# pengfeidip/pytorch-faster-rcnn

Measured on AMD Instinct MI355X. Metric: img/s FasterRCNN_R50_FPN 1000x600 fwd+loss, higher is better.
Workload: dtype f32; 1 GPU; configs/faster_rcnn_r50_fpn.py (BASELINE config 2) forward_train; conv_algorithms=MIOpen benchmarked (warmup, at most 32 tuning iterations per solver), trunk=hipGraph replay (backbone + neck + RPN head convs), global_batch=2, imgs_per_gpu=2, image=600x1000 padded 608x1024, parallelism=dp1, sampler=device, mode=fwd

## Files before the change

include/frcnn_amd.h:

```cpp
#ifndef FRCNN_AMD_H
#define FRCNN_AMD_H

#include <stddef.h>
#include <stdint.h>

#ifdef __cplusplus
extern "C" {
#endif

#define FRH_ABI_VERSION 3

#define FRH_OK 0
#define FRH_EINVAL (-1)
#define FRH_EUNSUPPORTED (-2)
#define FRH_ELAUNCH (-3)

#define FRH_MAX_LEVELS 8

int32_t frh_abi_version(void);
const char* frh_last_error(void);

#define FRH_DEVERR_SELECT_BARRIER 1
#define FRH_DEVERR_NMS_COLUMN 2
#define FRH_DEVERR_SAMPLER_BARRIER 4
// ... 213 lines not shown
                         int32_t channels, const float* rois, int64_t num_rois, int32_t pooled_h,
                         int32_t pooled_w, const float* grad_out, const int32_t* argmax, void* stream);

size_t frh_atss_workspace(int32_t batch, int32_t max_gts, int32_t num_levels, int32_t topk,
                          int64_t num_cells);
int32_t frh_atss_assign(int32_t batch, int32_t num_levels, const int32_t* grid_hw,
                        const float* strides, const float* anchors, int64_t anchor_ld,
                        const float* gts, int64_t gt_seg_stride, const int32_t* num_gts,
                        const int64_t* gt_labels, int32_t max_gts, const int32_t* img_hw,
                        int32_t topk, int64_t* cls, float* reg, float* ctr, void* workspace,
                        size_t ws_bytes, void* stream);

int32_t frh_bn_act(const float* x, const float* skip, float* y, const float* gamma,
                   const float* beta, const float* mean, const float* var, float eps,
                   int64_t n, int32_t c, int64_t hw, int32_t relu, void* stream);

int32_t frh_bn_act_maxpool(const float* x, float* y, const float* gamma, const float* beta, const float* mean,
                           const float* var, float eps, int64_t n, int32_t c, int32_t h, int32_t w, void* stream);

int32_t frh_conv1x1_bn_act(const float* x, const float* w, const float* skip, float* y, const float* gamma,
                           const float* beta, const float* mean, const float* var, float eps, int64_t n,
                           int32_t cin, int32_t cout, int64_t hw, int32_t relu, void* stream);

size_t frh_conv3x3_workspace(int32_t cin, int32_t cout);
int32_t frh_conv3x3_bias_act(const float* x, const float* w, const float* bias, float* y, float* workspace,
                             int64_t n, int32_t cin, int32_t cout, int32_t h, int32_t wd, int64_t sn, int64_t sy,
                             int64_t sx, int32_t relu, void* stream);
int32_t frh_conv3x3_bias_act_levels(int32_t num_levels, const void* const* xs, const void* const* weights,
                                    const void* const* biases, void* const* ys, float* workspace,
                                    size_t workspace_bytes, int64_t n, int32_t cin, int32_t cout,
                                    const int32_t* level_hw, const int64_t* level_strides, int32_t relu,
                                    void* stream);

size_t frh_roi_conv3x3_workspace(int32_t cin, int32_t cout);
int32_t frh_roi_conv3x3_bn_act(const float* x, const float* w, float* y, const float* gamma, const float* beta,
                               const float* mean, const float* var, float eps, int64_t r, int32_t cin,
                               int32_t cout, int32_t relu, float* workspace, void* stream);

int32_t frh_fpn_merge_nhwc(const float* lat, const int64_t* lat_strides, const float* bias, const float* up,
                           int32_t up_h, int32_t up_w, float* out, int32_t batch, int32_t channels, int32_t height,
                           int32_t width, void* stream);

size_t frh_bfp_argmax_elems(int32_t num_levels, int32_t refine_level, int32_t batch, int32_t channels,
                            const int32_t* level_hw);
int32_t frh_bfp_fwd(int32_t num_levels, int32_t refine_level, int32_t batch, int32_t channels,
                    const void* const* feats, const int32_t* level_hw, const int64_t* level_strides,
// ... 72 lines not shown
```

pytorch-faster-rcnn_amd/csrc/conv1x1.hip:

```cpp
#include "conv1x1_kernels.h"

using namespace frh;

extern "C" int32_t frh_conv1x1_bn_act(const float* x, const float* w, const float* skip, float* y, const float* gamma,
                                      const float* beta, const float* mean, const float* var, float eps, int64_t n,
                                      int32_t cin, int32_t cout, int64_t hw, int32_t relu, void* stream) {
  return conv1x1_launch(conv1x1_pick_step(cin), x, w, skip, y, gamma, beta, mean, var, eps, n, cin, cout, hw, relu,
                        stream);
}
```

pytorch-faster-rcnn_amd/csrc/conv1x1_kernels.h:

```cpp
#pragma once
#include <math.h>

#include "common.h"

namespace frh {

typedef float f32x16 __attribute__((ext_vector_type(16)));

constexpr int kCxThreads = 256;
constexpr int kCxTile = 64;
constexpr int kCxXcds = 8;

struct Conv1x1Args {
  const float* x;
  const float* w;
  const float* skip;
  float* y;
  const float* gamma;
  const float* beta;
  const float* mean;
  const float* var;
  float eps;
  int cin, cout;
  int64_t hw;
  int mt, pt;
  int64_t total;
  int64_t chunk;
  int relu;
};

template <int BK>
__global__ void __launch_bounds__(kCxThreads) conv1x1_bn_act_kernel(const Conv1x1Args a) {
  constexpr int T = kCxTile, PA = BK + 4, PB = T + 4, HK = BK / 2;
  constexpr int NV = T * (BK / 4) / kCxThreads;
  static_assert(NV == 1 || NV == 2, "staging registers are written out for one or two float4");
  constexpr int A_ROWS = kCxThreads / (BK / 4), B_ROWS = kCxThreads / (T / 4);
  __shared__ __attribute__((aligned(16))) float As[2][T * PA];
  __shared__ __attribute__((aligned(16))) float Bs[2][BK * PB];
  __shared__ float bn_s[T], bn_b[T];

  const int64_t wg = (int64_t)(blockIdx.x % kCxXcds) * a.chunk + blockIdx.x / kCxXcds;
  if (wg >= a.total) return;
  const int m_tile = (int)(wg % a.mt);
  const int64_t rest = wg / a.mt;
  const int p_tile = (int)(rest % a.pt);
  const int64_t img = rest / a.pt;
  const int m0 = m_tile * T;
  const int64_t p0 = (int64_t)p_tile * T;

  const int tid = threadIdx.x;
  const int lane = tid & 63, wave = tid >> 6;
  const int wm = wave >> 1, wn = wave & 1;
  const int h = lane >> 5, j = lane & 31;

  const bool bn = a.mean != nullptr;
  if (bn && tid < T) {
    const int c = m0 + tid;
    const float s = (a.gamma ? a.gamma[c] : 1.0f) / sqrtf(a.var[c] + a.eps);
    bn_s[tid] = s;
    bn_b[tid] = (a.beta ? a.beta[c] : 0.0f) - a.mean[c] * s;
  }

  const int a_row = tid / (BK / 4), a_q = tid % (BK / 4);
  const int b_row = tid / (T / 4), b_q = tid % (T / 4);
  const float* wp = a.w + (int64_t)(m0 + a_row) * a.cin + a_q * 4;
  const bool p_ok = p0 + b_q * 4 < a.hw;
  const float* xp = a.x + (img * a.cin + b_row) * a.hw + p0 + b_q * 4;
  const float4 z4 = make_float4(0.0f, 0.0f, 0.0f, 0.0f);
  float4 ra0, ra1 = z4, rb0 = z4, rb1 = z4;
#define FRH_CX_LOAD(k0)                                                                         \
  do {                                                                                          \
    ra0 = *reinterpret_cast<const float4*>(wp + (k0));                                          \
    if (NV > 1) ra1 = *reinterpret_cast<const float4*>(wp + (int64_t)A_ROWS * a.cin + (k0));    \
    if (p_ok) {                                                                                 \
      rb0 = *reinterpret_cast<const float4*>(xp + (int64_t)(k0)*a.hw);                          \
      if (NV > 1) rb1 = *reinterpret_cast<const float4*>(xp + (int64_t)((k0) + B_ROWS) * a.hw); \
    }                                                                                           \
  } while (0)

  f32x16 acc;
#pragma unroll
  for (int r = 0; r < 16; ++r) acc[r] = 0.0f;

  const int steps = a.cin / BK;
  FRH_CX_LOAD(0);
  for (int t = 0; t < steps; ++t) {
    const int buf = t & 1;
    *reinterpret_cast<float4*>(&As[buf][a_row * PA + a_q * 4]) = ra0;
    if (NV > 1) *reinterpret_cast<float4*>(&As[buf][(a_row + A_ROWS) * PA + a_q * 4]) = ra1;
    *reinterpret_cast<float4*>(&Bs[buf][b_row * PB + b_q * 4]) = rb0;
    if (NV > 1) *reinterpret_cast<float4*>(&Bs[buf][(b_row + B_ROWS) * PB + b_q * 4]) = rb1;
    __syncthreads();
    if (t + 1 < steps) FRH_CX_LOAD((t + 1) * BK);
#pragma unroll
    for (int q = 0; q < HK / 8; ++q) {
      const float* ap = &As[buf][(wm * 32 + j) * PA + h * HK + q * 8];
      const float4 lo = *reinterpret_cast<const float4*>(ap);
      const float4 hi = *reinterpret_cast<const float4*>(ap + 4);
      const float af[8] = {lo.x, lo.y, lo.z, lo.w, hi.x, hi.y, hi.z, hi.w};
      float bf[8];
#pragma unroll
      for (int s = 0; s < 8; ++s) bf[s] = Bs[buf][(h * HK + q * 8 + s) * PB + wn * 32 + j];
#pragma unroll
      for (int s = 0; s < 8; ++s) acc = __builtin_amdgcn_mfma_f32_32x32x2f32(af[s], bf[s], acc, 0, 0, 0);
    }
  }
#undef FRH_CX_LOAD

  const int64_t p = p0 + wn * 32 + j;
  if (p >= a.hw) return;
  const int lrow = wm * 32 + 4 * h;
  const int64_t off = (img * a.cout + m0 + lrow) * a.hw + p;
  float k[16];
  if (a.skip) {
#pragma unroll
    for (int r = 0; r < 16; ++r) k[r] = a.skip[off + (int64_t)((r & 3) + 8 * (r >> 2)) * a.hw];
  }
#pragma unroll
  for (int r = 0; r < 16; ++r) {
    const int lr = lrow + (r & 3) + 8 * (r >> 2);
    float v = acc[r];
    if (bn) v = v * bn_s[lr] + bn_b[lr];
    if (a.skip) v = v + k[r];
    if (a.relu) v = fmaxf(v, 0.0f);
    a.y[off + (int64_t)((r & 3) + 8 * (r >> 2)) * a.hw] = v;
  }
}

inline int conv1x1_pick_step(int32_t cin) { return cin >= 128 && cin % 32 == 0 ? 32 : 16; }

inline int32_t conv1x1_launch(int step, const float* x, const float* w, const float* skip, float* y,
                              const float* gamma, const float* beta, const float* mean, const float* var, float eps,
                              int64_t n, int32_t cin, int32_t cout, int64_t hw, int32_t relu, void* stream) {
  FRH_REQUIRE(n >= 0 && cin >= 1 && cout >= 1 && hw >= 0, "bad sizes");
  if (n == 0 || hw == 0) return FRH_OK;
  FRH_REQUIRE(x && w && y, "null pointer argument");
  FRH_REQUIRE((mean == nullptr) == (var == nullptr), "mean and var must both be given or both be NULL");
  FRH_REQUIRE(hw % 4 == 0, "plane size %lld must be a multiple of 4", (long long)hw);
  FRH_REQUIRE(cin % 16 == 0 && cout % kCxTile == 0, "cin %d must be a multiple of 16 and cout %d of 64", cin, cout);
  FRH_REQUIRE(((uintptr_t)x | (uintptr_t)y | (uintptr_t)skip | (uintptr_t)w) % 16 == 0,
              "tensors must be 16-byte aligned");
  FRH_REQUIRE(y != x && y != skip, "y must not alias x or skip");
  FRH_REQUIRE((step == 16 || step == 32) && cin % step == 0, "step %d does not fit cin %d", step, cin);
  Conv1x1Args a;
  a.x = x, a.w = w, a.skip = skip, a.y = y, a.gamma = gamma, a.beta = beta, a.mean = mean, a.var = var, a.eps = eps;
  a.cin = cin, a.cout = cout, a.hw = hw, a.relu = relu;
  a.mt = cout / kCxTile;
  const int64_t pt = (hw + kCxTile - 1) / kCxTile;
  FRH_REQUIRE(pt < ((int64_t)1 << 31), "too many pixel tiles");
  a.pt = (int)pt;
  a.total = (int64_t)a.mt * pt * n;
  a.chunk = (a.total + kCxXcds - 1) / kCxXcds;
  FRH_REQUIRE(a.chunk * kCxXcds < ((int64_t)1 << 31), "too many blocks");
  const dim3 grid((unsigned)(a.chunk * kCxXcds)), block(kCxThreads);
  if (step == 32)
    hipLaunchKernelGGL((conv1x1_bn_act_kernel<32>), grid, block, 0, as_stream(stream), a);
  else
    hipLaunchKernelGGL((conv1x1_bn_act_kernel<16>), grid, block, 0, as_stream(stream), a);
  return check_launch("frh_conv1x1_bn_act");
}

}
```

pytorch-faster-rcnn_amd/frcnn_amd/_lib.py:

```python
import ctypes
import os

import torch

_HERE = os.path.dirname(os.path.abspath(__file__))
LIB_PATH = os.path.join(_HERE, 'libfrcnn_amd.so')

c_i32, c_i64, c_f32, c_f64 = ctypes.c_int32, ctypes.c_int64, ctypes.c_float, ctypes.c_double
c_u64, c_size, c_vp = ctypes.c_uint64, ctypes.c_size_t, ctypes.c_void_p
P = ctypes.POINTER

SIGNATURES = {
    'frh_abi_version': (c_i32, []),
    'frh_last_error': (ctypes.c_char_p, []),
    'frh_anchor_grid': (c_i32, [c_i32, P(c_i32), P(c_f32), c_vp, c_vp, c_i32, c_i32, c_vp, c_i64, c_vp]),
    'frh_inside_mask': (c_i32, [c_vp, c_i64, c_i32, P(c_i32), P(c_i32), c_i32, c_i32, c_i32, c_i32, c_vp, c_vp]),
    'frh_iou_table': (c_i32, [c_vp, c_i64, c_i64, c_vp, c_i64, c_i64, c_vp, c_vp]),
    'frh_elem_iou': (c_i32, [c_vp, c_i64, c_vp, c_i64, c_i64, c_vp, c_vp]),
    'frh_maxiou_assign_zero_bytes': (c_size, [c_i32, c_i32]),
    'frh_maxiou_assign_workspace': (c_size, [c_i32, c_i32, c_i64]),
    'frh_maxiou_assign': (c_i32, [c_i32, c_vp, c_i64, c_i64, c_vp, c_vp, c_i64, c_vp, c_i64, c_i64, c_vp,
                                  c_f32, c_f32, c_f32, c_vp, c_i64, c_vp, c_i64, c_i64, c_i32, c_vp, c_size,
                                  c_vp]),
    'frh_sample_workspace': (c_size, [c_i32, c_i64]),
# ... 49 lines not shown
    'frh_roi_rows': (c_i32, [c_i32, c_vp, c_i64, c_i64, c_i32, P(c_i64), c_f32, c_i32, c_vp, c_vp, c_vp]),
    'frh_roi_rows_dev': (c_i32, [c_i32, c_vp, c_i64, c_i64, c_vp, c_f32, c_i32, c_vp, c_vp, c_vp]),
    'frh_roi_align_fwd': (c_i32, [c_i32, P(c_vp), P(c_i32), P(c_f32), c_i32, c_i32, c_i32, c_vp, c_vp, c_i64,
                                  c_i32, c_i32, c_i32, c_i32, c_vp, c_vp]),
    'frh_roi_align_bwd': (c_i32, [c_i32, P(c_vp), P(c_i32), P(c_f32), c_i32, c_i32, c_i32, c_vp, c_vp, c_i64,
                                  c_i32, c_i32, c_i32, c_i32, c_vp, c_vp]),
    'frh_roi_align_fwd_strided': (c_i32, [c_i32, P(c_vp), P(c_i32), P(c_i64), P(c_f32), c_i32, c_i32, c_vp,
                                          c_vp, c_i64, c_i32, c_i32, c_i32, c_i32, c_vp, c_vp]),
    'frh_roi_align_fwd_strided_timed': (c_i32, [c_i32, P(c_vp), P(c_i32), P(c_i64), P(c_f32), c_i32, c_i32, c_vp,
                                                c_vp, c_i64, c_i32, c_i32, c_i32, c_i32, c_vp, c_vp, c_vp, c_vp,
                                                c_vp]),
    'frh_roi_align_bwd_strided': (c_i32, [c_i32, P(c_vp), P(c_i32), P(c_i64), P(c_f32), c_i32, c_i32, c_vp,
                                          c_vp, c_i64, c_i32, c_i32, c_i32, c_i32, c_vp, c_vp]),
    'frh_roi_align_bwd_fixed': (c_i32, [c_i32, P(c_vp), P(c_vp), P(c_i32), P(c_i64), P(c_f32), c_i32, c_i32, c_vp,
                                        c_vp, c_i64, c_i32, c_i32, c_i32, c_i32, c_vp, c_vp, c_vp]),
    'frh_roi_pool_fwd': (c_i32, [c_vp, P(c_i64), c_i32, c_i32, c_i32, c_f32, c_vp, c_i64, c_i32, c_i32, c_vp,
                                 c_vp, c_vp]),
    'frh_roi_pool_bwd': (c_i32, [c_vp, P(c_i64), c_i32, c_i32, c_i32, c_vp, c_i64, c_i32, c_i32, c_vp, c_vp,
                                 c_vp]),
    'frh_atss_workspace': (c_size, [c_i32, c_i32, c_i32, c_i32, c_i64]),
    'frh_bn_act': (c_i32, [c_vp, c_vp, c_vp, c_vp, c_vp, c_vp, c_vp, c_f32, c_i64, c_i32, c_i64, c_i32, c_vp]),
    'frh_conv1x1_bn_act': (c_i32, [c_vp, c_vp, c_vp, c_vp, c_vp, c_vp, c_vp, c_vp, c_f32, c_i64, c_i32, c_i32, c_i64, c_i32,
                                   c_vp]),
    'frh_conv3x3_workspace': (c_size, [c_i32, c_i32]),
    'frh_conv3x3_bias_act': (c_i32, [c_vp, c_vp, c_vp, c_vp, c_vp, c_i64, c_i32, c_i32, c_i32, c_i32, c_i64, c_i64, c_i64,
                                     c_i32, c_vp]),
    'frh_conv3x3_bias_act_levels': (c_i32, [c_i32, P(c_vp), P(c_vp), P(c_vp), P(c_vp), c_vp, c_size, c_i64, c_i32, c_i32,
                                            P(c_i32), P(c_i64), c_i32, c_vp]),
    'frh_roi_conv3x3_workspace': (c_size, [c_i32, c_i32]),
    'frh_roi_conv3x3_bn_act': (c_i32, [c_vp, c_vp, c_vp, c_vp, c_vp, c_vp, c_vp, c_f32, c_i64, c_i32, c_i32, c_i32, c_vp,
                                       c_vp]),
    'frh_bn_act_maxpool': (c_i32, [c_vp, c_vp, c_vp, c_vp, c_vp, c_vp, c_f32, c_i64, c_i32, c_i32, c_i32, c_vp]),
    'frh_loss_workspace': (c_size, []),
    'frh_fpn_merge_nhwc': (c_i32, [c_vp, P(c_i64), c_vp, c_vp, c_i32, c_i32, c_vp, c_i32, c_i32, c_i32, c_i32, c_vp]),
    'frh_bfp_argmax_elems': (c_size, [c_i32, c_i32, c_i32, c_i32, P(c_i32)]),
    'frh_bfp_fwd': (c_i32, [c_i32, c_i32, c_i32, c_i32, P(c_vp), P(c_i32), P(c_i64), c_vp, P(c_vp), c_vp, c_i64,
                            c_vp]),
    'frh_bfp_bwd': (c_i32, [c_i32, c_i32, c_i32, c_i32, P(c_vp), P(c_i32), P(c_i64), c_vp, c_i64, c_vp, P(c_vp),
                            c_vp]),
    'frh_bias_act_nhwc': (c_i32, [c_vp, c_vp, c_i64, c_i32, c_i32, c_vp]),
    'frh_image_preprocess': (c_i32, [c_vp, c_i32, P(c_i64), P(c_i32), P(c_i32), P(c_i32), P(c_f32), P(c_f32), c_i32,
                                     c_vp, c_i32, c_i32, c_vp]),
    'frh_cls_loss_fwd': (c_i32, [c_i32, c_vp, c_i64, c_i64, c_i64, c_i64, c_vp, c_i32, c_f32, c_f32, c_vp, c_vp,
                                 c_vp, c_size, c_vp]),
    'frh_cls_loss_bwd': (c_i32, [c_i32, c_vp, c_i64, c_i64, c_i64, c_i64, c_vp, c_i32, c_f32, c_f32, c_vp, c_vp,
                                 c_i64, c_i64, c_vp]),
# ... 87 lines not shown
```

pytorch-faster-rcnn_amd/frcnn_amd/backbones.py:

```python
import logging

import torch
from torch import nn

from .ops import bn_act, bn_act_maxpool, conv1x1_bn_act

_STAGE_BLOCKS = {50: (3, 4, 6, 3), 101: (3, 4, 23, 3), 152: (3, 8, 36, 3)}
_STAGE_WIDTH = (64, 256, 512, 1024, 2048)


def _conv_bn(cin, cout, k, stride=1, pad=0):
    return nn.Conv2d(cin, cout, k, stride=stride, padding=pad, bias=False), nn.BatchNorm2d(cout)


class Bottleneck(nn.Module):

    def __init__(self, in_channels, out_channels, downsample=False):
        super().__init__()
        mid = out_channels // 4
        first_stage = in_channels * 4 == out_channels
        stride = 2 if (downsample and not first_stage) else 1
        self.conv1, self.bn1 = _conv_bn(in_channels, mid, 1)
        self.conv2, self.bn2 = _conv_bn(mid, mid, 3, stride=stride, pad=1)
        self.conv3, self.bn3 = _conv_bn(mid, out_channels, 1)
        self.relu = nn.ReLU(inplace=True)
        self.do_downsample = downsample
        if downsample:
            self.downsample = nn.Sequential(*_conv_bn(in_channels, out_channels, 1, stride=stride))

    def forward(self, x):
        y = conv1x1_bn_act(self.conv1, self.bn1, x)
        y = bn_act(self.conv2(y), self.bn2)
        skip = conv1x1_bn_act(self.downsample[0], self.downsample[1], x, relu=False) if self.do_downsample else x
        return conv1x1_bn_act(self.conv3, self.bn3, y, skip=skip)


class ResNet(nn.Module):
    def __init__(self, depth=50, frozen_stages=1, out_layers=(1, 2, 3, 4), pretrained=True):
        super().__init__()
        if depth not in _STAGE_BLOCKS:
            raise AssertionError('unsupported ResNet depth {}'.format(depth))
        self.depth = depth
        self.pretrained = pretrained
        self.frozen_stages = frozen_stages
        self.out_layers = tuple(out_layers)
        self.conv_cfg = _STAGE_BLOCKS[depth]
        self.conv1, self.bn1 = _conv_bn(3, 64, 7, stride=2, pad=3)
        self.relu = nn.ReLU(inplace=True)
        self.maxpool = nn.MaxPool2d(kernel_size=3, stride=2, padding=1)
        for s, nblk in enumerate(self.conv_cfg):
            cin, cout = _STAGE_WIDTH[s], _STAGE_WIDTH[s + 1]
            blocks = [Bottleneck(cin, cout, True)] + [Bottleneck(cout, cout) for _ in range(nblk - 1)]
            setattr(self, 'layer{}'.format(s + 1), nn.Sequential(*blocks))

    def forward(self, x):
        x = bn_act_maxpool(self.conv1(x), self.bn1, self.maxpool)
        outs = []
# ... 60 lines not shown
```

pytorch-faster-rcnn_amd/frcnn_amd/heads/rpn_head.py:

```python
import logging

import torch
from torch import nn

from .. import ops
from ..bbox import PropBatch
from ..utils import init_module_normal
from .anchor_head import AnchorHead


class LazyPropList(PropBatch):

    def __init__(self, buffer, counts_dev, what='boxes'):
        super().__init__()
        self.buffer = buffer
        self.counts_dev = counts_dev
        self._what = what
        self._n = buffer.shape[0]
        self._done = False

    def _materialise(self):
        if not self._done:
            self._done = True
            counts = self.counts_dev.cpu().tolist()
# ... 20 lines not shown
    def __init__(self, in_channels, feat_channels, anchor_scales=(8,), anchor_ratios=(0.5, 1.0, 2.0),
                 anchor_strides=(4, 8, 16, 32, 64), anchor_center_lt=False, target_means=(0.0, 0.0, 0.0, 0.0),
                 target_stds=(1.0, 1.0, 1.0, 1.0), loss_cls=None, loss_bbox=None):
        self.in_channels = in_channels
        self.feat_channels = feat_channels
        super().__init__(num_classes=2, anchor_scales=anchor_scales, anchor_ratios=anchor_ratios,
                         anchor_strides=anchor_strides, anchor_center_lt=anchor_center_lt,
                         target_means=target_means, target_stds=target_stds, loss_cls=loss_cls,
                         loss_bbox=loss_bbox)
        self.init_layers()

    def init_layers(self):
        self.conv = nn.Conv2d(self.in_channels, self.feat_channels, kernel_size=3, stride=1, padding=1)
        self.relu = nn.ReLU(inplace=True)
        self.classifier = nn.Conv2d(self.feat_channels, self.num_anchors * self.cls_channels, kernel_size=1)
        self.regressor = nn.Conv2d(self.feat_channels, self.num_anchors * 4, kernel_size=1)

    def init_weights(self):
        for m in (self.conv, self.classifier, self.regressor):
            init_module_normal(m, mean=0.0, std=0.01)

    def forward(self, xs):
        hidden = ops.conv3x3_bias_act_levels(self.conv, xs, relu=True)
        return [self.classifier(h) for h in hidden], [self.regressor(h) for h in hidden]

    def predict_bboxes_from_output(self, cls_outs, reg_outs, img_metas, test_cfg):
        with torch.no_grad():
            dev = cls_outs[0].device
            grid_sizes = [tuple(c.shape[-2:]) for c in cls_outs]
            anchors = self._flat_anchors(grid_sizes, dev)
            img_hw = [tuple(float(v) for v in m['img_shape'][:2]) for m in img_metas]
            min_sizes = [float(m['scale_factor'] * test_cfg.min_bbox_size) for m in img_metas]
            boxes, scores, counts = ops.rpn_proposals(
                [c.detach() for c in cls_outs], [r.detach() for r in reg_outs], anchors, self.num_anchors,
                self.cls_channels, self.target_means, self.target_stds, img_hw, min_sizes, int(test_cfg.pre_nms),
                int(test_cfg.post_nms), int(test_cfg.max_num), float(test_cfg.nms_iou))
        props = LazyPropList(boxes, counts, 'boxes')
        scs = LazyPropList(scores, counts, 'scores')
        return [props, scs, [None] * len(img_metas)]

    def predict_single_image(self, level_cls_outs, level_reg_outs, level_anchors, img_meta, test_cfg):
        p, s, _ = self.predict_bboxes_from_output([c.unsqueeze(0) for c in level_cls_outs],
                                                  [r.unsqueeze(0) for r in level_reg_outs], [img_meta], test_cfg)
        return p[0], s[0], None
```

pytorch-faster-rcnn_amd/frcnn_amd/ops.py:

```python
import ctypes
import os
import warnings

import numpy as np
import torch
from torch import nn

from . import _lib
from ._lib import call as _call, ptr, stream_of, i32_array, i64_array, f32_array, ptr_array, workspace


def call(name, *args):
    try:
        _call(name, *args)
    except RuntimeError:
        _drop_zero_workspaces()
        raise


def _drop_zero_workspaces():
    for ws in (_ASSIGN_WS, _SAMPLE_WS, _LOSS_WS):
        ws.clear()


# ... 1027 lines not shown
    return torch.is_grad_enabled() and any(t is not None and t.requires_grad for t in tensors)


_CONV1X1_EXCLUDED = frozenset([(512, 128), (512, 256), (1024, 256), (1024, 512), (2048, 512)])


def conv1x1_fused_ok(conv, bn, x, skip=None):
    if not (x.is_cuda and x.dtype == torch.float32 and x.dim() == 4 and x.is_contiguous()
            and not bn.training and conv.bias is None and conv.weight.dtype == torch.float32
            and conv.kernel_size == (1, 1) and conv.stride == (1, 1) and conv.padding == (0, 0)
            and conv.dilation == (1, 1) and conv.groups == 1 and conv.weight.is_contiguous()):
        return False
    cout, cin, hw = conv.out_channels, conv.in_channels, x.shape[2] * x.shape[3]
    if x.shape[1] != cin or hw % 4 or cin % 16 or cout % 64 or (x.data_ptr() | conv.weight.data_ptr()) % 16 \
            or (cin, cout) in _CONV1X1_EXCLUDED:
        return False
    if skip is not None and not (skip.is_cuda and skip.dtype == torch.float32 and skip.is_contiguous()
                                 and skip.shape == (x.shape[0], cout, x.shape[2], x.shape[3])
                                 and skip.data_ptr() % 16 == 0):
        return False
    return not _needs_grad(x, skip, conv.weight, bn.weight, bn.bias)


def conv1x1_bn_act(conv, bn, x, skip=None, relu=True):
    if not conv1x1_fused_ok(conv, bn, x, skip):
        return bn_act(conv(x), bn, skip=skip, relu=relu)
    n, _, h, w = x.shape
    y = torch.empty(n, conv.out_channels, h, w, dtype=torch.float32, device=x.device)
    call('frh_conv1x1_bn_act', ptr(x), ptr(conv.weight), ptr(skip), ptr(y), ptr(bn.weight), ptr(bn.bias),
         ptr(bn.running_mean), ptr(bn.running_var), float(bn.eps), n, conv.in_channels, conv.out_channels, h * w,
         int(bool(relu)), stream_of(x))
    return y


def roi_conv3x3_fused_ok(conv, bn, x):
    if not (x.is_cuda and x.dtype == torch.float32 and x.dim() == 4 and x.shape[2:] == (7, 7) and x.is_contiguous()
            and not bn.training and bn.running_mean is not None and conv.bias is None and conv.weight.dtype == torch.float32
            and conv.kernel_size == (3, 3) and conv.stride == (1, 1) and conv.padding == (1, 1)
            and conv.dilation == (1, 1) and conv.groups == 1 and conv.padding_mode == 'zeros'
            and conv.weight.is_contiguous()):
        return False
    cout, cin = conv.out_channels, conv.in_channels
    if x.shape[1] != cin or cin % 16 or cout % 64 or (x.data_ptr() | conv.weight.data_ptr()) % 16:
        return False
    return not _needs_grad(x, conv.weight, bn.weight, bn.bias)


def roi_conv3x3_bn_act(conv, bn, x, relu=True):
    if not roi_conv3x3_fused_ok(conv, bn, x):
        y = bn(conv(x))
        return torch.relu(y) if relu else y
    r = x.shape[0]
    y = torch.empty(r, conv.out_channels, 7, 7, dtype=torch.float32, device=x.device)
    ws = torch.empty(9 * conv.in_channels * conv.out_channels, dtype=torch.float32, device=x.device)
    call('frh_roi_conv3x3_bn_act', ptr(x), ptr(conv.weight), ptr(y), ptr(bn.weight), ptr(bn.bias),
# ... 340 lines not shown
```

Measured before the change: 400.3 img/s.

## Fuse bottleneck BN2 into conv3, add stride-2 1x1 projection and fused RPN head

Folds the post-conv2 batchnorm+ReLU into the input staging of the conv3 1x1 kernel, so the separate bn_act pass over the activation disappears. Adds a stride-2 gather form of the 1x1 conv for downsample projections, which avoids the MIOpen strided conv plus a separate BN. Replaces the per-level RPN classifier and regressor convs with one multi-level kernel that computes both outputs. The cost is more template variants, per-block recomputation of the per-channel BN scales, and half-wasted strided loads in the s2 path. Some shapes fall back through exclusion lists.

```diff
diff --git a/include/frcnn_amd.h b/include/frcnn_amd.h
--- a/include/frcnn_amd.h
+++ b/include/frcnn_amd.h
@@ -259,6 +259,21 @@
                            const float* beta, const float* mean, const float* var, float eps, int64_t n,
                            int32_t cin, int32_t cout, int64_t hw, int32_t relu, void* stream);
 
+int32_t frh_conv1x1_bn_act_pre(const float* x, const float* w, const float* skip, float* y, const float* gamma,
+                               const float* beta, const float* mean, const float* var, float eps,
+                               const float* pre_gamma, const float* pre_beta, const float* pre_mean,
+                               const float* pre_var, float pre_eps, int32_t pre_relu, int64_t n, int32_t cin,
+                               int32_t cout, int64_t hw, int32_t relu, void* stream);
+
+int32_t frh_conv1x1_s2_bn_act(const float* x, const float* w, const float* skip, float* y, const float* gamma,
+                              const float* beta, const float* mean, const float* var, float eps, int64_t n,
+                              int32_t cin, int32_t cout, int32_t h, int32_t wd, int32_t relu, void* stream);
+
+int32_t frh_rpn_head1x1_levels(int32_t num_levels, const void* const* xs, void* const* cls_outs,
+                               void* const* reg_outs, const float* w_cls, const float* b_cls, const float* w_reg,
+                               const float* b_reg, int64_t n, int32_t cin, int32_t c_cls, int32_t c_reg,
+                               const int32_t* level_hw, const int64_t* level_strides, void* stream);
+
 size_t frh_conv3x3_workspace(int32_t cin, int32_t cout);
 int32_t frh_conv3x3_bias_act(const float* x, const float* w, const float* bias, float* y, float* workspace,
                              int64_t n, int32_t cin, int32_t cout, int32_t h, int32_t wd, int64_t sn, int64_t sy,
diff --git a/pytorch-faster-rcnn_amd/csrc/conv1x1.hip b/pytorch-faster-rcnn_amd/csrc/conv1x1.hip
--- a/pytorch-faster-rcnn_amd/csrc/conv1x1.hip
+++ b/pytorch-faster-rcnn_amd/csrc/conv1x1.hip
@@ -8,3 +8,29 @@
   return conv1x1_launch(conv1x1_pick_step(cin), x, w, skip, y, gamma, beta, mean, var, eps, n, cin, cout, hw, relu,
                         stream);
 }
+
+extern "C" int32_t frh_conv1x1_bn_act_pre(const float* x, const float* w, const float* skip, float* y,
+                                          const float* gamma, const float* beta, const float* mean, const float* var,
+                                          float eps, const float* pre_gamma, const float* pre_beta,
+                                          const float* pre_mean, const float* pre_var, float pre_eps, int32_t pre_relu,
+                                          int64_t n, int32_t cin, int32_t cout, int64_t hw, int32_t relu,
+                                          void* stream) {
+  FRH_REQUIRE(pre_mean && pre_var, "the input BN needs its mean and var");
+  Conv1x1Input in;
+  in.pre_gamma = pre_gamma, in.pre_beta = pre_beta, in.pre_mean = pre_mean, in.pre_var = pre_var;
+  in.pre_eps = pre_eps, in.pre_relu = pre_relu;
+  return conv1x1_launch(conv1x1_pick_step(cin), x, w, skip, y, gamma, beta, mean, var, eps, n, cin, cout, hw, relu,
+                        stream, &in, "frh_conv1x1_bn_act_pre");
+}
+
+extern "C" int32_t frh_conv1x1_s2_bn_act(const float* x, const float* w, const float* skip, float* y,
+                                         const float* gamma, const float* beta, const float* mean, const float* var,
+                                         float eps, int64_t n, int32_t cin, int32_t cout, int32_t h, int32_t wd,
+                                         int32_t relu, void* stream) {
+  FRH_REQUIRE(h >= 1 && wd >= 1, "bad sizes");
+  FRH_REQUIRE(wd % 8 == 0, "input width %d must be a multiple of 8 (output width a multiple of 4)", wd);
+  Conv1x1Input in;
+  in.in_h = h, in.in_w = wd;
+  return conv1x1_launch(conv1x1_pick_step(cin), x, w, skip, y, gamma, beta, mean, var, eps, n, cin, cout,
+                        (int64_t)((h + 1) / 2) * (wd / 2), relu, stream, &in, "frh_conv1x1_s2_bn_act");
+}
diff --git a/pytorch-faster-rcnn_amd/csrc/conv1x1_kernels.h b/pytorch-faster-rcnn_amd/csrc/conv1x1_kernels.h
--- a/pytorch-faster-rcnn_amd/csrc/conv1x1_kernels.h
+++ b/pytorch-faster-rcnn_amd/csrc/conv1x1_kernels.h
@@ -10,6 +10,7 @@
 constexpr int kCxThreads = 256;
 constexpr int kCxTile = 64;
 constexpr int kCxXcds = 8;
+constexpr int kCxPreMax = 512;
 
 struct Conv1x1Args {
   const float* x;
@@ -27,9 +28,23 @@
   int64_t total;
   int64_t chunk;
   int relu;
+  const float* pre_gamma;
+  const float* pre_beta;
+  const float* pre_mean;
+  const float* pre_var;
+  float pre_eps;
+  int pre_relu;
+  int64_t in_hw;
+  int in_w, w_out;
 };
 
-template <int BK>
+__device__ __forceinline__ float4 conv1x1_pre(float4 v, float s, float b, int relu) {
+  float4 r = make_float4(v.x * s + b, v.y * s + b, v.z * s + b, v.w * s + b);
+  if (relu) r = make_float4(fmaxf(r.x, 0.0f), fmaxf(r.y, 0.0f), fmaxf(r.z, 0.0f), fmaxf(r.w, 0.0f));
+  return r;
+}
+
+template <int BK, bool PRE = false, bool S2 = false>
 __global__ void __launch_bounds__(kCxThreads) conv1x1_bn_act_kernel(const Conv1x1Args a) {
   constexpr int T = kCxTile, PA = BK + 4, PB = T + 4, HK = BK / 2;
   constexpr int NV = T * (BK / 4) / kCxThreads;
@@ -38,6 +53,7 @@
   __shared__ __attribute__((aligned(16))) float As[2][T * PA];
   __shared__ __attribute__((aligned(16))) float Bs[2][BK * PB];
   __shared__ float bn_s[T], bn_b[T];
+  __shared__ float pre_s[PRE ? kCxPreMax : 1], pre_b[PRE ? kCxPreMax : 1];
 
   const int64_t wg = (int64_t)(blockIdx.x % kCxXcds) * a.chunk + blockIdx.x / kCxXcds;
   if (wg >= a.total) return;
@@ -61,20 +77,41 @@
     bn_b[tid] = (a.beta ? a.beta[c] : 0.0f) - a.mean[c] * s;
   }
 
+  if constexpr (PRE) {
+    for (int c = tid; c < a.cin; c += kCxThreads) {
+      const float s = (a.pre_gamma ? a.pre_gamma[c] : 1.0f) / sqrtf(a.pre_var[c] + a.pre_eps);
+      pre_s[c] = s;
+      pre_b[c] = (a.pre_beta ? a.pre_beta[c] : 0.0f) - a.pre_mean[c] * s;
+    }
+    __syncthreads();
+  }
+
   const int a_row = tid / (BK / 4), a_q = tid % (BK / 4);
   const int b_row = tid / (T / 4), b_q = tid % (T / 4);
   const float* wp = a.w + (int64_t)(m0 + a_row) * a.cin + a_q * 4;
   const bool p_ok = p0 + b_q * 4 < a.hw;
-  const float* xp = a.x + (img * a.cin + b_row) * a.hw + p0 + b_q * 4;
+  const float* xp;
+  if constexpr (S2) {
+    const int64_t pq = p0 + b_q * 4, oy = pq / a.w_out, ox = pq - oy * a.w_out;
+    xp = a.x + (img * a.cin + b_row) * a.in_hw + 2 * oy * a.in_w + 2 * ox;
+  } else {
+    xp = a.x + (img * a.cin + b_row) * a.hw + p0 + b_q * 4;
+  }
+  const int64_t xs = S2 ? a.in_hw : a.hw;
   const float4 z4 = make_float4(0.0f, 0.0f, 0.0f, 0.0f);
   float4 ra0, ra1 = z4, rb0 = z4, rb1 = z4;
+  float4 rc0 = z4, rc1 = z4;
 #define FRH_CX_LOAD(k0)                                                                         \
   do {                                                                                          \
     ra0 = *reinterpret_cast<const float4*>(wp + (k0));                                          \
     if (NV > 1) ra1 = *reinterpret_cast<const float4*>(wp + (int64_t)A_ROWS * a.cin + (k0));    \
     if (p_ok) {                                                                                 \
-      rb0 = *reinterpret_cast<const float4*>(xp + (int64_t)(k0)*a.hw);                          \
-      if (NV > 1) rb1 = *reinterpret_cast<const float4*>(xp + (int64_t)((k0) + B_ROWS) * a.hw); \
+      rb0 = *reinterpret_cast<const float4*>(xp + (int64_t)(k0)*xs);                            \
+      if (NV > 1) rb1 = *reinterpret_cast<const float4*>(xp + (int64_t)((k0) + B_ROWS) * xs);   \
+      if (S2) {                                                                                 \
+        rc0 = *reinterpret_cast<const float4*>(xp + (int64_t)(k0)*xs + 4);                      \
+        if (NV > 1) rc1 = *reinterpret_cast<const float4*>(xp + (int64_t)((k0) + B_ROWS) * xs + 4); \
+      }                                                                                         \
     }                                                                                           \
   } while (0)
 
@@ -88,8 +125,15 @@
     const int buf = t & 1;
     *reinterpret_cast<float4*>(&As[buf][a_row * PA + a_q * 4]) = ra0;
     if (NV > 1) *reinterpret_cast<float4*>(&As[buf][(a_row + A_ROWS) * PA + a_q * 4]) = ra1;
-    *reinterpret_cast<float4*>(&Bs[buf][b_row * PB + b_q * 4]) = rb0;
-    if (NV > 1) *reinterpret_cast<float4*>(&Bs[buf][(b_row + B_ROWS) * PB + b_q * 4]) = rb1;
+    float4 vb0 = S2 ? make_float4(rb0.x, rb0.z, rc0.x, rc0.z) : rb0;
+    float4 vb1 = S2 ? make_float4(rb1.x, rb1.z, rc1.x, rc1.z) : rb1;
+    if constexpr (PRE) {
+      const int c = t * BK + b_row;
+      vb0 = conv1x1_pre(vb0, pre_s[c], pre_b[c], a.pre_relu);
+      if (NV > 1) vb1 = conv1x1_pre(vb1, pre_s[c + B_ROWS], pre_b[c + B_ROWS], a.pre_relu);
+    }
+    *reinterpret_cast<float4*>(&Bs[buf][b_row * PB + b_q * 4]) = vb0;
+    if (NV > 1) *reinterpret_cast<float4*>(&Bs[buf][(b_row + B_ROWS) * PB + b_q * 4]) = vb1;
     __syncthreads();
     if (t + 1 < steps) FRH_CX_LOAD((t + 1) * BK);
 #pragma unroll
@@ -129,9 +173,21 @@
 
 inline int conv1x1_pick_step(int32_t cin) { return cin >= 128 && cin % 32 == 0 ? 32 : 16; }
 
+struct Conv1x1Input {
+  const float* pre_gamma = nullptr;
+  const float* pre_beta = nullptr;
+  const float* pre_mean = nullptr;
+  const float* pre_var = nullptr;
+  float pre_eps = 0.0f;
+  int32_t pre_relu = 0;
+  int32_t in_h = 0, in_w = 0;
+};
+
 inline int32_t conv1x1_launch(int step, const float* x, const float* w, const float* skip, float* y,
                               const float* gamma, const float* beta, const float* mean, const float* var, float eps,
-                              int64_t n, int32_t cin, int32_t cout, int64_t hw, int32_t relu, void* stream) {
+                              int64_t n, int32_t cin, int32_t cout, int64_t hw, int32_t relu, void* stream,
+                              const Conv1x1Input* in = nullptr, const char* what = "frh_conv1x1_bn_act") {
+  const bool pre = in && in->pre_mean, s2 = in && in->in_w > 0;
   FRH_REQUIRE(n >= 0 && cin >= 1 && cout >= 1 && hw >= 0, "bad sizes");
   if (n == 0 || hw == 0) return FRH_OK;
   FRH_REQUIRE(x && w && y, "null pointer argument");
@@ -142,7 +198,22 @@
               "tensors must be 16-byte aligned");
   FRH_REQUIRE(y != x && y != skip, "y must not alias x or skip");
   FRH_REQUIRE((step == 16 || step == 32) && cin % step == 0, "step %d does not fit cin %d", step, cin);
+  FRH_REQUIRE(!(pre && s2), "the input BN and the stride-2 gather are separate forms");
   Conv1x1Args a;
+  a.pre_gamma = a.pre_beta = a.pre_mean = a.pre_var = nullptr, a.pre_eps = 0.0f, a.pre_relu = 0;
+  a.in_hw = 0, a.in_w = a.w_out = 0;
+  if (in && !s2) {
+    FRH_REQUIRE(in->pre_mean && in->pre_var, "the input BN needs its mean and var");
+    FRH_REQUIRE(cin <= kCxPreMax, "cin %d above the input BN form's bound %d", cin, kCxPreMax);
+    a.pre_gamma = in->pre_gamma, a.pre_beta = in->pre_beta, a.pre_mean = in->pre_mean, a.pre_var = in->pre_var;
+    a.pre_eps = in->pre_eps, a.pre_relu = in->pre_relu;
+  }
+  if (s2) {
+    FRH_REQUIRE(in->in_h >= 1 && in->in_w % 8 == 0,
+                "input width %d must be a multiple of 8 (output width a multiple of 4)", in->in_w);
+    FRH_REQUIRE(hw == (int64_t)((in->in_h + 1) / 2) * (in->in_w / 2), "output plane does not match the input");
+    a.in_hw = (int64_t)in->in_h * in->in_w, a.in_w = in->in_w, a.w_out = in->in_w / 2;
+  }
   a.x = x, a.w = w, a.skip = skip, a.y = y, a.gamma = gamma, a.beta = beta, a.mean = mean, a.var = var, a.eps = eps;
   a.cin = cin, a.cout = cout, a.hw = hw, a.relu = relu;
   a.mt = cout / kCxTile;
@@ -153,11 +224,21 @@
   a.chunk = (a.total + kCxXcds - 1) / kCxXcds;
   FRH_REQUIRE(a.chunk * kCxXcds < ((int64_t)1 << 31), "too many blocks");
   const dim3 grid((unsigned)(a.chunk * kCxXcds)), block(kCxThreads);
-  if (step == 32)
-    hipLaunchKernelGGL((conv1x1_bn_act_kernel<32>), grid, block, 0, as_stream(stream), a);
+#define FRH_CX_GO(PRE, S2)                                                                             \
+  do {                                                                                                 \
+    if (step == 32)                                                                                    \
+      hipLaunchKernelGGL((conv1x1_bn_act_kernel<32, PRE, S2>), grid, block, 0, as_stream(stream), a);  \
+    else                                                                                               \
+      hipLaunchKernelGGL((conv1x1_bn_act_kernel<16, PRE, S2>), grid, block, 0, as_stream(stream), a);  \
+  } while (0)
+  if (pre)
+    FRH_CX_GO(true, false);
+  else if (s2)
+    FRH_CX_GO(false, true);
   else
-    hipLaunchKernelGGL((conv1x1_bn_act_kernel<16>), grid, block, 0, as_stream(stream), a);
-  return check_launch("frh_conv1x1_bn_act");
-}
-
-}
+    FRH_CX_GO(false, false);
+#undef FRH_CX_GO
+  return check_launch(what);
+}
+
+}
diff --git a/pytorch-faster-rcnn_amd/csrc/rpn_head1x1.hip b/pytorch-faster-rcnn_amd/csrc/rpn_head1x1.hip
--- /dev/null
+++ b/pytorch-faster-rcnn_amd/csrc/rpn_head1x1.hip
@@ -0,0 +1,23 @@
+#include "rpn_head1x1_kernels.h"
+
+using namespace frh;
+
+extern "C" int32_t frh_rpn_head1x1_levels(int32_t num_levels, const void* const* xs, void* const* cls_outs,
+                                          void* const* reg_outs, const float* w_cls, const float* b_cls,
+                                          const float* w_reg, const float* b_reg, int64_t n, int32_t cin,
+                                          int32_t c_cls, int32_t c_reg, const int32_t* level_hw,
+                                          const int64_t* level_strides, void* stream) {
+  FRH_REQUIRE(num_levels >= 1 && num_levels <= kRhMaxLevels, "1 to %d levels, got %d", kRhMaxLevels, num_levels);
+  FRH_REQUIRE(xs && cls_outs && reg_outs && level_hw && level_strides, "null pointer argument");
+  RpnHeadLevelDesc d[kRhMaxLevels];
+  for (int i = 0; i < num_levels; ++i)
+    d[i] = {static_cast<const float*>(xs[i]),
+            static_cast<float*>(cls_outs[i]),
+            static_cast<float*>(reg_outs[i]),
+            level_hw[2 * i],
+            level_hw[2 * i + 1],
+            level_strides[3 * i],
+            level_strides[3 * i + 1],
+            level_strides[3 * i + 2]};
+  return rpn_head1x1_launch(num_levels, d, w_cls, b_cls, w_reg, b_reg, n, cin, c_cls, c_reg, stream);
+}
diff --git a/pytorch-faster-rcnn_amd/csrc/rpn_head1x1_kernels.h b/pytorch-faster-rcnn_amd/csrc/rpn_head1x1_kernels.h
--- /dev/null
+++ b/pytorch-faster-rcnn_amd/csrc/rpn_head1x1_kernels.h
@@ -0,0 +1,199 @@
+#pragma once
+#include "common.h"
+
+namespace frh {
+
+typedef float f32x4 __attribute__((ext_vector_type(4)));
+
+constexpr int kRhThreads = 256;
+constexpr int kRhPix = 64;
+constexpr int kRhCols = 16;
+constexpr int kRhKC = 128;
+constexpr int kRhMaxCin = 256;
+constexpr int kRhMaxLevels = 8;
+constexpr int kRhWP = kRhMaxCin + 4, kRhXP = kRhKC + 4;
+constexpr int kRhLoads = kRhPix * (kRhKC / 4) / kRhThreads;
+
+struct RpnHeadLevel {
+  const float* x;
+  float* cls;
+  float* reg;
+  int64_t sn, sy, sx;
+  int64_t pixels;
+  int32_t h, w;
+  int32_t first;
+};
+
+struct RpnHeadArgs {
+  RpnHeadLevel lv[kRhMaxLevels];
+  const float* w_cls;
+  const float* b_cls;
+  const float* w_reg;
+  const float* b_reg;
+  int32_t levels, cin, c_cls, c_reg;
+  int32_t total, per_wg;
+};
+
+__global__ void __launch_bounds__(kRhThreads) rpn_head1x1_kernel(const RpnHeadArgs a) {
+  __shared__ __attribute__((aligned(16))) float Ws[kRhCols * kRhWP];
+  __shared__ __attribute__((aligned(16))) float Xs[kRhPix * kRhXP];
+  __shared__ int64_t in_off[kRhPix];
+  __shared__ float bias_s[kRhCols];
+  __shared__ RpnHeadLevel lvs[kRhMaxLevels];
+
+  const int tid = threadIdx.x;
+  const int lane = tid & 63, wave = tid >> 6;
+  const int p = lane & 15, g = lane >> 4;
+  const float4 z4 = make_float4(0.0f, 0.0f, 0.0f, 0.0f);
+  const int cout = a.c_cls + a.c_reg;
+
+  for (int f = tid; f < kRhCols * (kRhMaxCin / 4); f += kRhThreads) {
+    const int co = f / (kRhMaxCin / 4), c = (f % (kRhMaxCin / 4)) * 4;
+    float4 v = z4;
+    if (c < a.cin && co < cout)
+      v = *reinterpret_cast<const float4*>(co < a.c_cls ? a.w_cls + (int64_t)co * a.cin + c
+                                                         : a.w_reg + (int64_t)(co - a.c_cls) * a.cin + c);
+    *reinterpret_cast<float4*>(&Ws[co * kRhWP + c]) = v;
+  }
+  if (tid < kRhCols) {
+    float b = 0.0f;
+    if (tid < a.c_cls)
+      b = a.b_cls ? a.b_cls[tid] : 0.0f;
+    else if (tid < cout)
+      b = a.b_reg ? a.b_reg[tid - a.c_cls] : 0.0f;
+    bias_s[tid] = b;
+  }
+
+#pragma unroll
+  for (int i = 0; i < kRhMaxLevels; ++i)
+    if (tid == i) {
+      lvs[i].x = a.lv[i].x, lvs[i].cls = a.lv[i].cls, lvs[i].reg = a.lv[i].reg;
+      lvs[i].sn = a.lv[i].sn, lvs[i].sy = a.lv[i].sy, lvs[i].sx = a.lv[i].sx, lvs[i].pixels = a.lv[i].pixels;
+      lvs[i].h = a.lv[i].h, lvs[i].w = a.lv[i].w, lvs[i].first = a.lv[i].first;
+    }
+
+  const int chunks = (a.cin + kRhKC - 1) / kRhKC;
+  const int tile_end = min(a.total, (int)(blockIdx.x + 1) * a.per_wg);
+  for (int tile = blockIdx.x * a.per_wg; tile < tile_end; ++tile) {
+    int li = 0;
+#pragma unroll
+    for (int i = 1; i < kRhMaxLevels; ++i)
+      if (i < a.levels && tile >= a.lv[i].first) li = i;
+
+    __syncthreads();
+    const RpnHeadLevel& L = lvs[li];
+    const int64_t lin0 = (int64_t)(tile - L.first) * kRhPix;
+    const float* const lx = L.x;
+    const int64_t pixels = L.pixels;
+    if (tid < kRhPix) {
+      const int64_t lin = lin0 + tid;
+      int64_t off = -1;
+      if (lin < pixels) {
+        const int64_t hw = (int64_t)L.h * L.w, img = lin / hw, rem = lin - img * hw;
+        const int64_t y = rem / L.w, x = rem - y * L.w;
+        off = img * L.sn + y * L.sy + x * L.sx;
+      }
+      in_off[tid] = off;
+    }
+    __syncthreads();
+
+    float4 rb[kRhLoads];
+    auto load = [&](int c0) {
+#pragma unroll
+      for (int i = 0; i < kRhLoads; ++i) {
+        const int f = i * kRhThreads + tid, row = f / (kRhKC / 4), ch = c0 + (f % (kRhKC / 4)) * 4;
+        const int64_t off = in_off[row];
+        float4 v = z4;
+        if (off >= 0 && ch < a.cin) v = *reinterpret_cast<const float4*>(lx + off + ch);
+        rb[i] = v;
+      }
+    };
+
+    f32x4 acc = {0.0f, 0.0f, 0.0f, 0.0f};
+    load(0);
+    for (int c = 0; c < chunks; ++c) {
+      if (c > 0) __syncthreads();
+#pragma unroll
+      for (int i = 0; i < kRhLoads; ++i) {
+        const int f = i * kRhThreads + tid;
+        *reinterpret_cast<float4*>(&Xs[(f / (kRhKC / 4)) * kRhXP + (f % (kRhKC / 4)) * 4]) = rb[i];
+      }
+      __syncthreads();
+      if (c + 1 < chunks) load((c + 1) * kRhKC);
+      const int groups = (min(kRhKC, a.cin - c * kRhKC) + 15) / 16;
+      const float* xr = &Xs[(wave * 16 + p) * kRhXP + 4 * g];
+      const float* wr = &Ws[p * kRhWP + c * kRhKC + 4 * g];
+      for (int j = 0; j < groups; ++j) {
+        const float4 xv = *reinterpret_cast<const float4*>(xr + 16 * j);
+        const float4 wv = *reinterpret_cast<const float4*>(wr + 16 * j);
+        acc = __builtin_amdgcn_mfma_f32_16x16x4f32(xv.x, wv.x, acc, 0, 0, 0);
+        acc = __builtin_amdgcn_mfma_f32_16x16x4f32(xv.y, wv.y, acc, 0, 0, 0);
+        acc = __builtin_amdgcn_mfma_f32_16x16x4f32(xv.z, wv.z, acc, 0, 0, 0);
+        acc = __builtin_amdgcn_mfma_f32_16x16x4f32(xv.w, wv.w, acc, 0, 0, 0);
+      }
+    }
+
+    const float b = bias_s[p];
+#pragma unroll
+    for (int r = 0; r < 4; ++r) {
+      const int64_t lin = lin0 + wave * 16 + 4 * g + r;
+      if (lin >= pixels) continue;
+      const float v = acc[r] + b;
+      if (p < a.c_cls)
+        L.cls[lin * a.c_cls + p] = v;
+      else if (p < cout)
+        L.reg[lin * a.c_reg + (p - a.c_cls)] = v;
+    }
+  }
+}
+
+struct RpnHeadLevelDesc {
+  const float* x;
+  float* cls;
+  float* reg;
+  int32_t h, w;
+  int64_t sn, sy, sx;
+};
+
+inline int32_t rpn_head1x1_launch(int32_t levels, const RpnHeadLevelDesc* d, const float* w_cls, const float* b_cls,
+                                  const float* w_reg, const float* b_reg, int64_t n, int32_t cin, int32_t c_cls,
+                                  int32_t c_reg, void* stream) {
+  FRH_REQUIRE(levels >= 1 && levels <= kRhMaxLevels, "1 to %d levels, got %d", kRhMaxLevels, levels);
+  FRH_REQUIRE(n >= 0 && n < (1 << 20) && cin >= 1 && c_cls >= 0 && c_reg >= 0 && c_cls + c_reg >= 1, "bad sizes");
+  FRH_REQUIRE(c_cls + c_reg <= kRhCols, "%d + %d output channels, at most %d together", c_cls, c_reg, kRhCols);
+  FRH_REQUIRE(cin % 8 == 0 && cin <= kRhMaxCin, "cin %d must be a multiple of 8 and at most %d", cin, kRhMaxCin);
+  FRH_REQUIRE((c_cls == 0 || w_cls) && (c_reg == 0 || w_reg), "null pointer argument");
+  FRH_REQUIRE(((uintptr_t)w_cls | (uintptr_t)w_reg) % 16 == 0, "tensors must be 16-byte aligned");
+  RpnHeadArgs a;
+  a.levels = 0, a.cin = cin, a.c_cls = c_cls, a.c_reg = c_reg;
+  a.w_cls = w_cls, a.b_cls = b_cls, a.w_reg = w_reg, a.b_reg = b_reg;
+  int64_t total = 0;
+  for (int i = 0; i < levels; ++i) {
+    const RpnHeadLevelDesc& s = d[i];
+    FRH_REQUIRE(s.h >= 0 && s.w >= 0, "bad sizes");
+    if (n == 0 || s.h == 0 || s.w == 0) continue;
+    FRH_REQUIRE(s.x && (c_cls == 0 || s.cls) && (c_reg == 0 || s.reg), "null pointer argument");
+    FRH_REQUIRE((uintptr_t)s.x % 16 == 0, "tensors must be 16-byte aligned");
+    const int64_t sn = n > 1 ? s.sn : 0, sy = s.h > 1 ? s.sy : 0, sx = s.w > 1 ? s.sx : 0;
+    FRH_REQUIRE(sn >= 0 && sy >= 0 && sx >= 0 && (sn | sy | sx) % 4 == 0,
+                "x strides must be non-negative multiples of 4 elements");
+    FRH_REQUIRE(s.cls != s.x && s.reg != s.x, "the outputs must not alias x");
+    RpnHeadLevel& L = a.lv[a.levels++];
+    L.x = s.x, L.cls = s.cls, L.reg = s.reg, L.sn = sn, L.sy = sy, L.sx = sx, L.h = s.h, L.w = s.w;
+    L.pixels = n * s.h * s.w;
+    FRH_REQUIRE(L.pixels < ((int64_t)1 << 31), "too many pixels in one level");
+    L.first = (int32_t)total;
+    total += (L.pixels + kRhPix - 1) / kRhPix;
+    FRH_REQUIRE(total < ((int64_t)1 << 30), "too many tiles");
+  }
+  if (a.levels == 0) return FRH_OK;
+  for (int i = a.levels; i < kRhMaxLevels; ++i) a.lv[i] = a.lv[0];
+  a.total = (int32_t)total;
+  const int cap = resident_capacity(reinterpret_cast<const void*>(rpn_head1x1_kernel), kRhThreads);
+  a.per_wg = cap > 0 ? (int32_t)((total + cap - 1) / cap) : 4;
+  const int64_t grid = (total + a.per_wg - 1) / a.per_wg;
+  hipLaunchKernelGGL(rpn_head1x1_kernel, dim3((unsigned)grid), dim3(kRhThreads), 0, as_stream(stream), a);
+  return check_launch("frh_rpn_head1x1_levels");
+}
+
+}
diff --git a/pytorch-faster-rcnn_amd/frcnn_amd/_lib.py b/pytorch-faster-rcnn_amd/frcnn_amd/_lib.py
--- a/pytorch-faster-rcnn_amd/frcnn_amd/_lib.py
+++ b/pytorch-faster-rcnn_amd/frcnn_amd/_lib.py
@@ -95,6 +95,12 @@
     'frh_bn_act': (c_i32, [c_vp, c_vp, c_vp, c_vp, c_vp, c_vp, c_vp, c_f32, c_i64, c_i32, c_i64, c_i32, c_vp]),
     'frh_conv1x1_bn_act': (c_i32, [c_vp, c_vp, c_vp, c_vp, c_vp, c_vp, c_vp, c_vp, c_f32, c_i64, c_i32, c_i32, c_i64, c_i32,
                                    c_vp]),
+    'frh_conv1x1_bn_act_pre': (c_i32, [c_vp, c_vp, c_vp, c_vp, c_vp, c_vp, c_vp, c_vp, c_f32, c_vp, c_vp, c_vp, c_vp,
+                                       c_f32, c_i32, c_i64, c_i32, c_i32, c_i64, c_i32, c_vp]),
+    'frh_conv1x1_s2_bn_act': (c_i32, [c_vp, c_vp, c_vp, c_vp, c_vp, c_vp, c_vp, c_vp, c_f32, c_i64, c_i32, c_i32,
+                                      c_i32, c_i32, c_i32, c_vp]),
+    'frh_rpn_head1x1_levels': (c_i32, [c_i32, P(c_vp), P(c_vp), P(c_vp), c_vp, c_vp, c_vp, c_vp, c_i64, c_i32, c_i32,
+                                       c_i32, P(c_i32), P(c_i64), c_vp]),
     'frh_conv3x3_workspace': (c_size, [c_i32, c_i32]),
     'frh_conv3x3_bias_act': (c_i32, [c_vp, c_vp, c_vp, c_vp, c_vp, c_i64, c_i32, c_i32, c_i32, c_i32, c_i64, c_i64, c_i64,
                                      c_i32, c_vp]),
diff --git a/pytorch-faster-rcnn_amd/frcnn_amd/backbones.py b/pytorch-faster-rcnn_amd/frcnn_amd/backbones.py
--- a/pytorch-faster-rcnn_amd/frcnn_amd/backbones.py
+++ b/pytorch-faster-rcnn_amd/frcnn_amd/backbones.py
@@ -3,7 +3,7 @@
 import torch
 from torch import nn
 
-from .ops import bn_act, bn_act_maxpool, conv1x1_bn_act
+from .ops import bn_act_maxpool, conv1x1_bn_act, conv1x1_s2_bn_act
 
 _STAGE_BLOCKS = {50: (3, 4, 6, 3), 101: (3, 4, 23, 3), 152: (3, 8, 36, 3)}
 _STAGE_WIDTH = (64, 256, 512, 1024, 2048)
@@ -30,9 +30,12 @@
 
     def forward(self, x):
         y = conv1x1_bn_act(self.conv1, self.bn1, x)
-        y = bn_act(self.conv2(y), self.bn2)
-        skip = conv1x1_bn_act(self.downsample[0], self.downsample[1], x, relu=False) if self.do_downsample else x
-        return conv1x1_bn_act(self.conv3, self.bn3, y, skip=skip)
+        y = self.conv2(y)
+        skip = x
+        if self.do_downsample:
+            proj = conv1x1_s2_bn_act if self.downsample[0].stride == (2, 2) else conv1x1_bn_act
+            skip = proj(self.downsample[0], self.downsample[1], x, relu=False)
+        return conv1x1_bn_act(self.conv3, self.bn3, y, skip=skip, pre_bn=self.bn2)
 
 
 class ResNet(nn.Module):
diff --git a/pytorch-faster-rcnn_amd/frcnn_amd/heads/rpn_head.py b/pytorch-faster-rcnn_amd/frcnn_amd/heads/rpn_head.py
--- a/pytorch-faster-rcnn_amd/frcnn_amd/heads/rpn_head.py
+++ b/pytorch-faster-rcnn_amd/frcnn_amd/heads/rpn_head.py
@@ -66,7 +66,7 @@
 
     def forward(self, xs):
         hidden = ops.conv3x3_bias_act_levels(self.conv, xs, relu=True)
-        return [self.classifier(h) for h in hidden], [self.regressor(h) for h in hidden]
+        return ops.rpn_head1x1_levels(self.classifier, self.regressor, hidden)
 
     def predict_bboxes_from_output(self, cls_outs, reg_outs, img_metas, test_cfg):
         with torch.no_grad():
diff --git a/pytorch-faster-rcnn_amd/frcnn_amd/ops.py b/pytorch-faster-rcnn_amd/frcnn_amd/ops.py
--- a/pytorch-faster-rcnn_amd/frcnn_amd/ops.py
+++ b/pytorch-faster-rcnn_amd/frcnn_amd/ops.py
@@ -1073,15 +1073,122 @@
     return not _needs_grad(x, skip, conv.weight, bn.weight, bn.bias)
 
 
-def conv1x1_bn_act(conv, bn, x, skip=None, relu=True):
+_CONV1X1_PRE_EXCLUDED = frozenset([(512, 2048)])
+_CONV1X1_S2_EXCLUDED = frozenset([(512, 1024), (1024, 2048)])
+_CONV1X1_PRE_MAX_CIN = 512
+
+
+def conv1x1_pre_fused_ok(conv, bn, x, pre_bn, skip=None):
+    return (conv1x1_fused_ok(conv, bn, x, skip) and not pre_bn.training and pre_bn.running_mean is not None
+            and pre_bn.num_features == conv.in_channels and conv.in_channels <= _CONV1X1_PRE_MAX_CIN
+            and (conv.in_channels, conv.out_channels) not in _CONV1X1_PRE_EXCLUDED
+            and not _needs_grad(pre_bn.weight, pre_bn.bias))
+
+
+def conv1x1_bn_act(conv, bn, x, skip=None, relu=True, pre_bn=None):
+    if pre_bn is not None and not conv1x1_pre_fused_ok(conv, bn, x, pre_bn, skip):
+        x, pre_bn = bn_act(x, pre_bn), None
     if not conv1x1_fused_ok(conv, bn, x, skip):
         return bn_act(conv(x), bn, skip=skip, relu=relu)
     n, _, h, w = x.shape
     y = torch.empty(n, conv.out_channels, h, w, dtype=torch.float32, device=x.device)
+    if pre_bn is not None:
+        call('frh_conv1x1_bn_act_pre', ptr(x), ptr(conv.weight), ptr(skip), ptr(y), ptr(bn.weight), ptr(bn.bias),
+             ptr(bn.running_mean), ptr(bn.running_var), float(bn.eps), ptr(pre_bn.weight), ptr(pre_bn.bias),
+             ptr(pre_bn.running_mean), ptr(pre_bn.running_var), float(pre_bn.eps), 1, n, conv.in_channels,
+             conv.out_channels, h * w, int(bool(relu)), stream_of(x))
+        return y
     call('frh_conv1x1_bn_act', ptr(x), ptr(conv.weight), ptr(skip), ptr(y), ptr(bn.weight), ptr(bn.bias),
          ptr(bn.running_mean), ptr(bn.running_var), float(bn.eps), n, conv.in_channels, conv.out_channels, h * w,
          int(bool(relu)), stream_of(x))
     return y
+
+
+def conv1x1_s2_fused_ok(conv, bn, x):
+    if not (x.is_cuda and x.dtype == torch.float32 and x.dim() == 4 and x.is_contiguous()
+            and not bn.training and bn.running_mean is not None and conv.bias is None
+            and conv.weight.dtype == torch.float32 and conv.kernel_size == (1, 1) and conv.stride == (2, 2)
+            and conv.padding == (0, 0) and conv.dilation == (1, 1) and conv.groups == 1
+            and conv.weight.is_contiguous()):
+        return False
+    cout, cin = conv.out_channels, conv.in_channels
+    if x.shape[1] != cin or x.shape[0] == 0 or x.shape[2] == 0 or x.shape[3] == 0 or x.shape[3] % 8 or cin % 16 \
+            or cout % 64 or (x.data_ptr() | conv.weight.data_ptr()) % 16 or (cin, cout) in _CONV1X1_S2_EXCLUDED:
+        return False
+    return not _needs_grad(x, conv.weight, bn.weight, bn.bias)
+
+
+def conv1x1_s2_bn_act(conv, bn, x, relu=False):
+    if not conv1x1_s2_fused_ok(conv, bn, x):
+        return bn_act(conv(x), bn, relu=relu)
+    n, _, h, w = x.shape
+    y = torch.empty(n, conv.out_channels, (h + 1) // 2, w // 2, dtype=torch.float32, device=x.device)
+    call('frh_conv1x1_s2_bn_act', ptr(x), ptr(conv.weight), None, ptr(y), ptr(bn.weight), ptr(bn.bias),
+         ptr(bn.running_mean), ptr(bn.running_var), float(bn.eps), n, conv.in_channels, conv.out_channels, h, w,
+         int(bool(relu)), stream_of(x))
+    return y
+
+
+_RPN_HEAD1X1_MAX_COUT = 16
+_RPN_HEAD1X1_MAX_CIN = 256
+
+
+def _plain_1x1(conv):
+    return (conv.kernel_size == (1, 1) and conv.stride == (1, 1) and conv.padding == (0, 0)
+            and conv.dilation == (1, 1) and conv.groups == 1 and conv.weight.dtype == torch.float32
+            and conv.weight.stride(0) == conv.in_channels and conv.weight.stride(1) == 1
+            and conv.weight.data_ptr() % 16 == 0
+            and (conv.bias is None or (conv.bias.dtype == torch.float32 and conv.bias.is_contiguous())))
+
+
+def rpn_head1x1_fused_ok(classifier, regressor, hidden):
+    hidden = list(hidden)
+    if not hidden or len(hidden) > 8 or not (_plain_1x1(classifier) and _plain_1x1(regressor)):
+        return False
+    cin = classifier.in_channels
+    if regressor.in_channels != cin or cin % 8 or cin > _RPN_HEAD1X1_MAX_CIN \
+            or classifier.out_channels + regressor.out_channels > _RPN_HEAD1X1_MAX_COUT:
+        return False
+    x0 = hidden[0]
+    for x in hidden:
+        if not (x.is_cuda and x.dtype == torch.float32 and x.dim() == 4 and x.device == x0.device
+                and x.shape[0] == x0.shape[0] and x.shape[1] == cin and x.numel() > 0 and x.stride(1) == 1
+                and (x.shape[2] * x.shape[3] == 1 or _suggests_channels_last(x))
+                and x.data_ptr() % 16 == 0 and all(s >= 0 and s % 4 == 0 for i, (d, s) in enumerate(zip(x.shape, x.stride())) if i != 1 and d > 1)
+                and x.shape[0] * x.shape[2] * x.shape[3] < 1 << 31):
+            return False
+    return not _needs_grad(classifier.weight, classifier.bias, regressor.weight, regressor.bias, *hidden)
+
+
+def _suggests_channels_last(t):
+    least = 0
+    if t.stride(1) == 0:
+        return False
+    for d in (1, 3, 2, 0):
+        if t.shape[d] == 0 or t.stride(d) < least or (d == 0 and least == t.stride(1)):
+            return False
+        least = t.stride(d) * max(t.shape[d], 1)
+    return True
+
+
+def rpn_head1x1_levels(classifier, regressor, hidden):
+    hidden = list(hidden)
+    if not rpn_head1x1_fused_ok(classifier, regressor, hidden):
+        return [classifier(h) for h in hidden], [regressor(h) for h in hidden]
+    n, dev, cin = hidden[0].shape[0], hidden[0].device, classifier.in_channels
+    cc, cr = classifier.out_channels, regressor.out_channels
+    def out(conv, x):
+        fmt = torch.channels_last if _suggests_channels_last(x) or _suggests_channels_last(conv.weight) \
+            else torch.contiguous_format
+        return torch.empty((n, conv.out_channels, x.shape[2], x.shape[3]), dtype=torch.float32, device=dev,
+                           memory_format=fmt)
+    cls = [out(classifier, x) for x in hidden]
+    reg = [out(regressor, x) for x in hidden]
+    call('frh_rpn_head1x1_levels', len(hidden), ptr_array(hidden), ptr_array(cls), ptr_array(reg),
+         ptr(classifier.weight), ptr(classifier.bias), ptr(regressor.weight), ptr(regressor.bias), n, cin, cc, cr,
+         i32_array([v for x in hidden for v in x.shape[2:]]),
+         i64_array([v for x in hidden for v in (x.stride(0), x.stride(2), x.stride(3))]), stream_of(hidden[0]))
+    return cls, reg
 
 
 def roi_conv3x3_fused_ok(conv, bn, x):
```

New measurement: 414.9 img/s (median of 6 runs). 3.6% higher.
